# PacificBiosciences/portello

Measured on AMD Instinct MI355X. Metric: lifted HiFi reads/sec (whole node), higher is better.
Workload: dtype int32; 1 GPU; wgs30x; reads_total=2000000, reads_this_rank=2000000, read_len_mean=15000, items_per_gpu=2065417, in_ops_per_gpu=62827345, out_ops_per_gpu=56590310, large_items_per_gpu=0, mid_items_per_gpu=0, retry_items_per_gpu=0, lane_items_per_gpu=2065417, heavy_lane_items_per_gpu=0, seq_fmt=bam4, parallelism=one read set, 20 Mb windows dealt to 1 ranks by input ops, gather=none, launched_by=single process

## Files before the change

portello_amd/csrc/lane_core.hpp:

```cpp
#pragma once
#include <plo_wave.hpp>
#include <stdint.h>

#include <type_traits>
#ifdef PLO_EMULATOR
#include <stdio.h>
#include <stdlib.h>
#endif

#include "lift_core.hpp"

#ifdef PLO_EMULATOR
#define PLO_MARK(s)
#else
#define PLO_MARK(s) asm volatile("; " s)
#endif

namespace plo {



#ifdef PLO_EMULATOR
struct __attribute__((packed, aligned(4))) Ops4 {
    uint32_t x, y, z, w;
};
#else
typedef uint32_t Ops4 __attribute__((ext_vector_type(4), aligned(4)));
#endif
struct LaneOut {
    uint32_t *R = nullptr;
    int no = 0;
    uint32_t acc = 0;
    int lead_shift = 0;
    bool seen_m = false;
    bool pairs = false;
    bool ovf = false;
    uint16_t *H = nullptr;
    int extra = 0;
};
PLO_DEV int wrap_add(int a, int b) { return (int)((unsigned)a + (unsigned)b); }
PLO_DEV bool b_is_match(int t) { return ((0x181u >> t) & 1u) != 0u; }
PLO_DEV bool b_is_indel(int t) { return (unsigned)(t - 1) < 2u; }
PLO_DEV bool b_ref_cons(int t) { return ((0x18Du >> t) & 1u) != 0u; }
PLO_DEV bool b_read_cons(int t) { return ((0x1B3u >> t) & 1u) != 0u; }

constexpr int H16_MAX = 8191, H16_CHUNKS = 8;
constexpr int H16_ALLOW = 4;
PLO_DEV uint32_t h16_dec(uint32_t h) { return ((h >> 3) << 4) | (h & 7u); }
PLO_DEV uint32_t h16_enc(int t, uint32_t len) { return (len << 3) | (uint32_t)t; }

template <int ST, bool H16>
PLO_DEV void lane_flush(LaneOut &o, bool flush, int wlim) {
    const int at = (int)(o.acc & 15u);
    if constexpr (!H16) {
        const bool ok = o.no < wlim;
        if (flush & ok) o.R[o.no * ST] = o.acc;
        o.ovf = o.ovf | (flush & !ok);
        o.no += flush ? 1 : 0;
    } else {
        static_assert(ST == 1, "H16 regions are lane-contiguous");
        const uint32_t len = o.acc >> 4;
        const bool ok = o.no < wlim;
        if (flush & ok) o.H[o.no] = (uint16_t)h16_enc(at, len < (uint32_t)H16_MAX ? len : (uint32_t)H16_MAX);
        o.ovf = o.ovf | (flush & !ok);
        o.no += flush ? 1 : 0;
        const bool big = flush & (len > (uint32_t)H16_MAX);
        if (wv::ballot(big) != 0ull) {
            uint32_t rest = big ? len - (uint32_t)H16_MAX : 0u;
#pragma unroll
            for (int c = 1; c < H16_CHUNKS; ++c) {
                const bool more = rest > 0u;
                const uint32_t part = rest < (uint32_t)H16_MAX ? rest : (uint32_t)H16_MAX;
                const bool okc = o.no < wlim;
                if (more & okc) o.H[o.no] = (uint16_t)h16_enc(at, part);
                o.ovf = o.ovf | (more & !okc);
                o.no += more ? 1 : 0;
                o.extra += more ? 1 : 0;
                rest -= part;
            }
            o.ovf = o.ovf | (rest > 0u);
        }
    }
}
template <bool PAD = true, int ST = 1, bool H16 = false>
PLO_DEV void lane_push(LaneOut &o, bool on, int t, int L, int wlim) {
    if constexpr (ST != 1) on = on & !o.ovf;
    const bool lead = on & !o.seen_m;
    const bool drop_d = lead & (t == OP_D);
    o.lead_shift += drop_d ? L : 0;
    t = (lead & (t == OP_I)) ? (int)OP_S : t;
    o.seen_m = o.seen_m | (on & b_is_match(t));
    const bool live = on & !drop_d & (L > 0);
    const int at = (int)(o.acc & 15u);
    const bool same = live & (t == at);
    const bool flush = live & !same & (o.acc >= 16u);
    o.pairs = o.pairs | (flush & b_is_indel(at) & b_is_indel(t));
    lane_flush<ST, H16>(o, flush, wlim);
    const uint32_t add = (PAD && t == OP_P) ? 0u : ((uint32_t)L << 4);
    o.acc = same ? o.acc + add : (live ? mk_op(t, L) : o.acc);
}
template <bool H16 = false>
PLO_DEV void lane_out_finish(LaneOut &o, bool on, int wlim) {
    lane_flush<1, H16>(o, on & (o.acc >= 16u), wlim);
    const bool fix0 = on & !o.ovf & o.seen_m;
    if constexpr (H16) {
        int lm = o.no - 1;
        {
            bool look = fix0 & (lm >= 0);
            while (wv::ballot(look) != 0ull) {
                const uint32_t c = o.H[look ? lm : 0];
                const bool hit = look & b_is_match((int)(c & 7u));
                look = look & !hit & (lm > 0);
                lm -= (look) ? 1 : 0;
            }
        }
        const bool fix = fix0 & (lm + 1 < o.no);
        LaneOut o2;
        o2.H = o.H;
        o2.no = lm + 1;
        o2.seen_m = true;
        int i = lm + 1, cont = 0, prev_t = -1;
        while (wv::ballot(fix & (i < o.no)) != 0ull) {
            const bool act = fix & (i < o.no);
            const uint32_t c = h16_dec(o.H[act ? i : 0]);
            int t = op_type(c);
            const int L = op_len(c);
            i += act ? 1 : 0;
            cont += (act & (t == prev_t)) ? 1 : 0;
            prev_t = act ? t : prev_t;
            const bool keep = act & (t != OP_D);
            t = (t == OP_I) ? (int)OP_S : t;
            lane_push<true, 1, true>(o2, keep, t, L, i);
        }
        lane_flush<1, true>(o2, fix & (o2.acc >= 16u), o.no);
        o.no = fix ? o2.no : o.no;
        o.extra = fix ? o.extra - cont + o2.extra : o.extra;
    } else {
        int lm = o.no - 1;
        {
            bool look = fix0 & (lm >= 0);
            while (wv::ballot(look) != 0ull) {
                const uint32_t c = o.R[look ? lm : 0];
                const bool hit = look & b_is_match(op_type(c));
                look = look & !hit & (lm > 0);
                lm -= (look) ? 1 : 0;
            }
        }
        const bool fix = fix0 & (lm + 1 < o.no);
        int i = lm + 1, w = lm + 1;
        uint32_t run = 0;
        while (wv::ballot(fix & (i < o.no)) != 0ull) {
            const bool act = fix & (i < o.no);
            const uint32_t c = o.R[act ? i : 0];
            int t = op_type(c);
            const int L = op_len(c);
            i += act ? 1 : 0;
            const bool keep = act & (t != OP_D);
            t = (t == OP_I) ? (int)OP_S : t;
            const bool same = keep & (run >= 16u) & (t == (int)(run & 15u));
            const bool flush = keep & !same & (run >= 16u);
            if (flush) o.R[w] = run;
            w += flush ? 1 : 0;
            const uint32_t add = (t == OP_P) ? 0u : ((uint32_t)L << 4);
            run = same ? run + add : (keep ? mk_op(t, L) : run);
        }
        {
            const bool flush = fix & (run >= 16u);
            if (flush) o.R[w] = run;
            w += flush ? 1 : 0;
            o.no = fix ? w : o.no;
        }
    }
}

struct XW16 {
    Ops4 r4, q4;
    uint32_t r1, q1;
    int rsh, qsh, jmin;
};
PLO_DEV bool xw16_issue(bool on, const uint8_t *ref, int ref_len, int r0, const ReadSeq &rd, int q0, const uint8_t *safe, XW16 &w, bool &miss) {
    bool ok = on & (r0 >= 0) & (q0 >= 0) & (q0 <= rd.len - 16);
    const int rsh = (int)(((unsigned)(uintptr_t)ref + (unsigned)r0) & 3u);
    ok = ok & (r0 - rsh >= 0) & (r0 - rsh <= ref_len - 20);
    const int jmin = rd.flip ? rd.len - q0 - 16 : q0;
    const bool bam4 = rd.fmt != PLO_SEQ_ASCII;
    int b0 = bam4 ? (jmin >> 1) : jmin;
    miss = false;
    if (rd.fmt == PLO_SEQ_BAM4_SPARSE) {
        const int j0 = ok ? jmin : 0, j1 = ok ? jmin + 15 : 0;
        const int g0 = j0 >> 5, g1 = j1 >> 5;
        const PLO_GLOBAL uint32_t *hdr = (const PLO_GLOBAL uint32_t *)(ok ? rd.p : safe);
        const uint32_t m0 = hdr[2 * (g0 >> 5)], rk0 = hdr[2 * (g0 >> 5) + 1], m1 = hdr[2 * (g1 >> 5)];
        const bool present = (((m0 >> (g0 & 31)) & (m1 >> (g1 & 31))) & 1u) != 0u;
        const unsigned rank = rk0 + (unsigned)__builtin_popcount(m0 & ((1u << (g0 & 31)) - 1u));
        const long long off = (long long)rd.data + (long long)rank * 16 + ((j0 >> 1) & 15);
        const bool bad = !present | (rank > 0x3ffffffu) | (off + (g1 - g0) * 16 + 20 > (long long)rd.hi);
        miss = ok & bad;
        ok = ok & !bad;
        b0 = (int)off;
    }
    const int qsh = (int)(((unsigned)(uintptr_t)rd.p + (unsigned)b0) & 3u);
    ok = ok & (b0 - qsh >= rd.lo) & (b0 - qsh + 20 <= rd.hi);
#ifdef PLO_EXP_PROBE_NOMEM
    const PLO_GLOBAL uint32_t *pr = (const PLO_GLOBAL uint32_t *)safe;
    const PLO_GLOBAL uint32_t *pq = (const PLO_GLOBAL uint32_t *)safe;
#else
    const PLO_GLOBAL uint32_t *pr = (const PLO_GLOBAL uint32_t *)(ok ? ref + (r0 - rsh) : safe);
    const PLO_GLOBAL uint32_t *pq = (const PLO_GLOBAL uint32_t *)(ok ? rd.p + (b0 - qsh) : safe);
#endif
    w.r4 = *(const PLO_GLOBAL Ops4 *)pr;
    w.r1 = pr[4];
    w.q4 = *(const PLO_GLOBAL Ops4 *)pq;
    w.q1 = pq[4];
    w.rsh = rsh;
    w.qsh = qsh;
    w.jmin = jmin;
    return ok;
}
PLO_DEV void xw16_decode(const ReadSeq &rd, const XW16 &wx, unsigned X[4]) {
    struct {
        unsigned wr[5], wq[5];
        int rsh, qsh, jmin;
    } w = {{wx.r4.x, wx.r4.y, wx.r4.z, wx.r4.w, wx.r1}, {wx.q4.x, wx.q4.y, wx.q4.z, wx.q4.w, wx.q1}, wx.rsh, wx.qsh, wx.jmin};
    const bool bam4 = rd.fmt != PLO_SEQ_ASCII;
    unsigned D[4];
    if (bam4) {
        unsigned S[5];
#pragma unroll
        for (int q = 0; q < 3; ++q) {
            unsigned Q = wv::align_bytes(w.wq[q + 1], w.wq[q], (unsigned)w.qsh);
            unsigned H = (Q >> 4) & 0x0f0f0f0fu, L = Q & 0x0f0f0f0fu;
            S[2 * q] = wv::perm_bytes(L, H, 0x05010400u);
            if (2 * q + 1 < 5) S[2 * q + 1] = wv::perm_bytes(L, H, 0x07030602u);
        }
        const unsigned par = (unsigned)(w.jmin & 1);
        const unsigned long long lo = rd.flip ? 0x4e4e4e434e47544eull : 0x565352474d43413dull;
        const unsigned long long hi = rd.flip ? 0x4e4e4e4e4e4e4e41ull : 0x4e42444b48595754ull;
#pragma unroll
        for (int v = 0; v < 4; ++v) {
            unsigned T = wv::align_bytes(S[v + 1], S[v], par);
            unsigned idx = T & 0x07070707u;
            unsigned dl = wv::perm_bytes((unsigned)(lo >> 32), (unsigned)lo, idx);
            unsigned dh = wv::perm_bytes((unsigned)(hi >> 32), (unsigned)hi, idx);
            unsigned mk = ((T >> 3) & 0x01010101u) * 0xffu;
            D[v] = (dh & mk) | (dl & ~mk);
        }
    } else {
#pragma unroll
        for (int v = 0; v < 4; ++v) {
            D[v] = wv::align_bytes(w.wq[v + 1], w.wq[v], (unsigned)w.qsh);
            if (rd.flip) D[v] = comp4(D[v]);
        }
    }
#pragma unroll
    for (int u = 0; u < 4; ++u) {
        unsigned R = wv::align_bytes(w.wr[u + 1], w.wr[u], (unsigned)w.rsh);
        unsigned B = rd.flip ? wv::perm_bytes(0u, D[3 - u], 0x00010203u) : D[u];
        X[u] = R ^ B;
    }
}

struct LaneProbe {
    XW16 w;
    int re = 0, qe = 0, maxk = 0;
    bool async_ok = false;
    bool miss = false;
};
PLO_DEV void lane_probe_arm(LaneProbe &p, bool on, int ref_len, int rs, int del, const ReadSeq &rd, int qs, int ins, int bound, bool &panic) {
    const int re = rs + del, qe = qs + ins;
    const int max_left = wv::imin(rs, qs);
    int maxk = wv::imin(max_left, bound);
    const bool bad = (max_left > 0) & ((re - 1 >= ref_len) | (qe - 1 >= rd.len));
    panic = panic | (on & bad);
    maxk = (bad | !on) ? 0 : maxk;
    p.re = re;
    p.qe = qe;
    p.maxk = maxk;
}
PLO_DEV void lane_probe_load(LaneProbe &p, bool on, const uint8_t *ref, int ref_len, const ReadSeq &rd, const uint8_t *safe) {
    p.async_ok = xw16_issue(on & (p.maxk > 0), ref, ref_len, p.re - 16, rd, p.qe - 16, safe, p.w, p.miss);
}
PLO_DEV int match_run_back_from(const uint8_t *ref, int ref_len, int re, ReadSeq &rd, int qe, int maxk, int k, int &probes) {
    while (k < maxk) {
        unsigned X[4];
        if (!xor_window16(ref, ref_len, re - k - 16, rd, qe - k - 16, X)) break;
        int n = wv::imin(16, maxk - k);
        int m = wv::imin(zero_bytes_from_top(X), n);
        probes += wv::imin(m + 1, n);
        k += m;
        if (m < n) return k;
    }
    while (k < maxk) {
        int n = wv::imin(8, maxk - k);
        int a[8], b[8];
#pragma unroll
        for (int j = 0; j < 8; ++j) {
            int jj = j < n ? j : 0;
            a[j] = ((const PLO_GLOBAL uint8_t *)ref)[re - 1 - k - jj];
            b[j] = read_base(rd, qe - 1 - k - jj);
        }
        int adv = n;
#pragma unroll
        for (int j = 7; j >= 0; --j)
            if (j < n && a[j] != b[j]) adv = j;
        probes += wv::imin(adv + 1, n);
        k += adv;
        if (adv < n) break;
    }
    return k;
}
PLO_DEV int top_zero_bytes(const unsigned X[4]) {
    const unsigned long long hi = ((unsigned long long)X[3] << 32) | X[2], lo = ((unsigned long long)X[1] << 32) | X[0];
    const int zh = hi ? (__builtin_clzll(hi) >> 3) : 8, zl = lo ? (__builtin_clzll(lo) >> 3) : 8;
    return hi ? zh : 8 + zl;
}
PLO_DEV int lane_probe_finish(const LaneProbe &p, bool on, const uint8_t *ref, int ref_len, ReadSeq &rd, int &probes) {
    unsigned X[4];
    xw16_decode(rd, p.w, X);
    const int n = wv::imin(16, p.maxk);
    const int m = wv::imin(top_zero_bytes(X), n);
    rd.miss = rd.miss | (on & p.miss);
    const bool live = on & (p.maxk > 0) & !p.miss;
    const bool fast = live & p.async_ok;
    int h = fast ? m : 0;
    probes += fast ? wv::imin(m + 1, n) : 0;
    const bool more = live & ((!p.async_ok) | ((m == n) & (n < p.maxk)));
    if (wv::ballot(more) != 0ull) {
        if (more) h = match_run_back_from(ref, ref_len, p.re, rd, p.qe, p.maxk, h, probes);
    }
    return h;
}

constexpr int LANE_RW = 20, LANE_WW = 28;
constexpr int LANE_WIN_DWORDS = LANE_RW + LANE_WW;
constexpr int LANE_WIN_MARGIN = 8;
constexpr int LANE_REGION_PAD = LANE_RW + 4;
struct LaneWin {
    uint32_t *G = nullptr;
    uint32_t *rw = nullptr, *ww = nullptr;
    int rbase = 0, wbase = 0;
};
PLO_DEV void win_fill(LaneWin &w, bool on, int idx) {
    if (on) {
        w.rbase = idx;
        Ops4 v[LANE_RW / 4];
#pragma unroll
        for (int q = 0; q < LANE_RW / 4; ++q) v[q] = *(const PLO_GLOBAL Ops4 *)(w.G + idx + 4 * q);
#pragma unroll
        for (int q = 0; q < LANE_RW / 4; ++q) {
            w.rw[(4 * q) * 64] = v[q].x;
            w.rw[(4 * q + 1) * 64] = v[q].y;
            w.rw[(4 * q + 2) * 64] = v[q].z;
            w.rw[(4 * q + 3) * 64] = v[q].w;
        }
    }
}
PLO_DEV void win_fill_input(LaneWin &w, bool on, int idx, const uint32_t *src, int n_in, bool rev, int lo_ok, int hi_ok) {
    uint32_t a[LANE_RW];
    const uint32_t *qa[LANE_RW / 4];
    bool edge = false;
#pragma unroll
    for (int q = 0; q < LANE_RW / 4; ++q) {
        const int kq = idx + 4 * q;
        const bool want = on & (kq < n_in);
        const int gi = rev ? n_in - 4 - kq : kq;
        const bool inside = (gi >= lo_ok) & (gi + 4 <= hi_ok);
        edge = edge | (want & !inside);
        qa[q] = (want & inside) ? src + gi : (const uint32_t *)plo_safe_words;
    }
    if (wv::ballot(edge) == 0ull) {
        Ops4 v[LANE_RW / 4];
#pragma unroll
        for (int q = 0; q < LANE_RW / 4; ++q) v[q] = *(const PLO_GLOBAL Ops4 *)qa[q];
#pragma unroll
        for (int q = 0; q < LANE_RW / 4; ++q) {
            a[4 * q] = rev ? v[q].w : v[q].x;
            a[4 * q + 1] = rev ? v[q].z : v[q].y;
            a[4 * q + 2] = rev ? v[q].y : v[q].z;
            a[4 * q + 3] = rev ? v[q].x : v[q].w;
        }
    } else {
#pragma unroll
        for (int j = 0; j < LANE_RW; ++j) {
            a[j] = 0u;
            if (on && idx + j < n_in) a[j] = src[rev ? n_in - 1 - idx - j : idx + j];
        }
    }
    if (on) {
        w.rbase = idx;
#pragma unroll
        for (int j = 0; j < LANE_RW; ++j) w.rw[j * 64] = (idx + j < n_in) ? a[j] : 0u;
    }
}
PLO_DEV void win_flush(LaneWin &w, bool on, int end) {
    if (on) {
        const int cnt = end - w.wbase;
        uint32_t *const dst = w.G + w.wbase;
#pragma unroll
        for (int q = 0; q < LANE_WW / 4; ++q) {
            Ops4 v;
            v.x = w.ww[(4 * q) * 64];
            v.y = w.ww[(4 * q + 1) * 64];
            v.z = w.ww[(4 * q + 2) * 64];
            v.w = w.ww[(4 * q + 3) * 64];
            if (4 * q + 3 < cnt) *(PLO_GLOBAL Ops4 *)(dst + 4 * q) = v;
        }
        const int n4 = cnt & ~3;
#pragma unroll
        for (int j = 0; j < 3; ++j)
            if (n4 + j < cnt) dst[n4 + j] = w.ww[(n4 + j) * 64];
        w.wbase = end;
    }
}

constexpr int LANE_KVS = 128;
constexpr int LANE_KVS_DWORDS = 2 * LANE_KVS;
constexpr int LANE_KVS_MAX = 512;
template <bool SP, bool WIN = false, bool NOSHIFT = false, bool STATS = true, bool H16 = false>
PLO_DEV void lane_tile(const DevIndex &ix, const DevBatch &bt, const DevWork &wk, uint32_t stages, uint32_t item_begin, int nit,
                       uint32_t *lds, int capw, int fixed_stride, WaveCtx &ctx, const uint32_t *list, bool have_g, uint32_t g_pre,
                       uint32_t *greg = nullptr, uint32_t *kvs = nullptr, int kvs_n = LANE_KVS) {
    static_assert(!(H16 && WIN), "16-bit ops: LDS regions only");
    const int lane = wv::lane();
    const bool has = lane < nit;
    const uint32_t g = have_g ? g_pre : (has ? list[item_begin + (uint32_t)lane] : 0u);
#ifdef PLO_PHASE_TIMING
    long long tlast = wv::clock();
#define PLO_LT(k)                     \
    {                                 \
        long long now_ = wv::clock(); \
        ctx.tph[k] += now_ - tlast;   \
        tlast = now_;                 \
    }
#define PLO_LC(k, v) ctx.tph[k] += (v);
#else
#define PLO_LT(k)
#define PLO_LC(k, v)
#endif

    int n_in = 0, n_m = 0, in_off = 0, pos1 = 0, kv0 = 0, kv1 = 0, W0 = 0, W1 = 0, seq_len = 0, shift_ref_len = 0;
    bool len_bad = false, rev = false, do_shift = false, flip = false;
    unsigned long long seq_off = 0, shift_ref = 0;
    if (has) {
        in_off = (int)wk.d.in_off[g];
        n_in = (int)wk.d.n_in[g];
        n_m = (int)wk.d.n_m[g];
        W0 = (int)wk.d.w0[g];
        W1 = (int)wk.d.w1[g];
        kv0 = (int)wk.d.kv0[g];
        kv1 = (int)wk.d.kv1[g];
        const uint32_t fl = wk.d.flags[g];
        pos1 = wk.d.pos1[g];
        seq_len = (int)wk.d.seq_len[g];
        const uint32_t read_len_in = wk.d.read_len[g];
        len_bad = read_len_in == 0xffffffffu || (uint32_t)seq_len != read_len_in;
        seq_off = wk.d.seq_off[g];
        shift_ref = wk.d.shift_ref[g];
        shift_ref_len = wk.d.shift_ref_len[g];
        rev = (fl & ITF_REV) != 0;
        flip = (fl & ITF_FLIP) != 0;
        const bool contig_fwd = (fl & ITF_CONTIG_FWD) != 0;
        do_shift = (stages & PLO_STAGE_LSHIFT) && (!(stages & PLO_STAGE_STRAND) || !contig_fwd);
    }
    const bool need_shift = do_shift;
    if constexpr (NOSHIFT) do_shift = false;
    const bool merges = do_shift || (stages & PLO_STAGE_LIFTOVER);
    const int n_ld = merges ? n_m : n_in;
    const int gap = has ? lane_region_gap(W0, W1) : 0;
    const int W = n_ld + gap + LANE_SLACK + (H16 ? H16_ALLOW : 0);
    const int W_dw = H16 ? (W + 1) >> 1 : W;

    int kvs_base = 0, kvs_cnt = 0;
    bool kv_lds = false, kvs_store = false;
    constexpr int KVS_Q = H16 ? LANE_KVS_MAX / 64 : LANE_KVS / 64;
    if constexpr (!H16) kvs_n = kvs_n < LANE_KVS ? kvs_n : LANE_KVS;
    KV kvs_e[KVS_Q];
#pragma unroll
    for (int q = 0; q < KVS_Q; ++q) kvs_e[q] = {0, 0};
    if (kvs != nullptr && (stages & PLO_STAGE_LIFTOVER)) {
        const int need_hi = wv::imin(kv1, W1 + 2);
        kvs_base = -wv::reduce_max(has ? -W0 : -IMAX);
        const int top = wv::reduce_max(has ? need_hi : 0);
        const int cnt = wv::imax(0, wv::imin(top - kvs_base, kvs_n));
        kv_lds = has & (need_hi <= kvs_base + cnt);
        kvs_cnt = cnt;
#pragma unroll
        for (int q = 0; q < KVS_Q; ++q)
            if (64 * q < kvs_n && lane + 64 * q < cnt) kvs_e[q] = ix.kv[kvs_base + lane + 64 * q];
        kvs_store = true;
    }

    bool pending = has;
    {
        const bool defer = has && (W_dw > (WIN ? fixed_stride - LANE_REGION_PAD : capw) || (NOSHIFT && need_shift));
        const unsigned long long dm = wv::ballot(defer);
        if (dm != 0ull) {
            int slot = 0;
            if (lane == 0) slot = (int)wv::atomic_add_global(&wk.counters[CNT_NRETRY], (unsigned long long)__builtin_popcountll(dm));
            slot = wv::bcast_first(slot);
            if (defer) {
                wk.retry_list[slot + __builtin_popcountll(dm & ((1ull << lane) - 1ull))] = g;
                wk.status[g] = (uint8_t)ITEM_NEED_BIG;
                pending = false;
            }
        }
    }

    while (wv::ballot(pending) != 0ull) {
        const int wv_ = pending ? W_dw : 0;
        const int incl = WIN ? 0 : wv::scan_add(wv_);
        const bool act0 = pending && (WIN || incl <= capw);
        pending = pending && !act0;
        uint32_t *R = WIN ? nullptr : lds + (act0 ? incl - wv_ : 0);
        uint16_t *const R16 = (uint16_t *)R;
        LaneWin win;
        if constexpr (WIN) {
            win.G = greg + (size_t)(has ? lane : 0) * (size_t)fixed_stride;
            win.rw = lds + lane;
            win.ww = lds + LANE_RW * 64 + lane;
        }
        wv::sync();

        int status = PLO_ITEM_LIFTED;
        bool alive = act0;
        bool shift_on = act0 && do_shift;
        if (shift_on && shift_ref == 0ull) {
            status = PLO_ITEM_PANIC;
            alive = false;
            shift_on = false;
        }
        bool ovf = false, panic = false;
        unsigned algo = 0;
        int cur_off = 0, n = 0;
        int nops = 0;
        constexpr int ST = WIN ? 64 : 1;
        auto rd_at = [&](int k, bool ok) -> uint32_t {
            if constexpr (WIN) return win.rw[ok ? (cur_off + k - win.rbase) * 64 : 0];
            else if constexpr (H16) return h16_dec(R16[cur_off + (ok ? k : 0)]);
            else return R[cur_off + (ok ? k : 0)];
        };
        const bool direct = WIN && (stages & PLO_STAGE_LIFTOVER) != 0u;
        const int n_cig_all = WIN ? (int)bt.seg_cigar_off[bt.n_segs] : 0;
        bool ext = false;
        auto rd_fill = [&](bool on, int idx) {
            if constexpr (WIN) {
                if (direct) {
                    if (wv::ballot(on & ext) != 0ull) win_fill_input(win, on & ext, idx, bt.cigar + in_off, n_in, rev, -in_off, n_cig_all - in_off);
                    if (wv::ballot(on & !ext) != 0ull) win_fill(win, on & !ext, idx);
                } else {
                    win_fill(win, on, idx);
                }
            }
        };
        auto rd_need = [&](int k, bool ok, bool stage_on) {
            if constexpr (WIN) {
                if (wv::ballot(ok & (cur_off + k - win.rbase >= LANE_RW)) != 0ull) rd_fill(stage_on, cur_off + k);
            }
        };
        auto wr_open = [&](LaneOut &o, int base) {
            if constexpr (WIN) {
                win.wbase = base;
                o.R = win.ww;
            } else if constexpr (H16) {
                o.H = R16 + base;
            } else {
                o.R = R + base;
            }
        };
        auto wr_room = [&](LaneOut &o, bool on, int base) {
            if constexpr (WIN) {
                if (wv::ballot(on & !o.ovf & (base + o.no - win.wbase > LANE_WW - LANE_WIN_MARGIN)) != 0ull) {
                    win_flush(win, on & !o.ovf, base + o.no);
                    o.R = win.ww - o.no * 64;
                }
            }
        };
        auto wr_finish = [&](LaneOut &o, bool on, int base, int wlim) {
            if constexpr (WIN) {
                win_flush(win, on & !o.ovf, base + o.no);
                o.R = win.G + base;
            }
            lane_out_finish<H16>(o, on, wlim);
        };
        int pos = pos1;
        ReadSeq rd = item_read_seq<SP>(bt, seq_off, seq_len, flip ? 1 : 0);
        PLO_LT(0)

        if (direct) {
            n = act0 ? n_in : 0;
            ext = act0;
        } else {
            const bool ld = act0;
            const bool merge = ld & merges;
            const int inb = shift_on ? W - n_ld - (H16 ? H16_ALLOW : 0) : gap;
            const int nmax = wv::reduce_max(ld ? n_in : 0);
            const int n_cig = (int)bt.seg_cigar_off[bt.n_segs];
            uint32_t run = 0;
            bool has_run = false;
            int w = 0;
            if constexpr (WIN) win.wbase = inb;
            bool ld_ovf = false;
            auto put = [&](bool on, uint32_t v) {
                if constexpr (WIN) {
                    if (on) win.ww[(inb + w - win.wbase) * 64] = v;
                } else if constexpr (H16) {
                    const uint32_t len = v >> 4;
                    const int vt = b_is_match((int)(v & 15u)) ? (int)OP_M : (int)(v & 15u);
                    const bool ok = inb + w < W;
                    if (on & ok) R16[inb + w] = (uint16_t)h16_enc(vt, len < (uint32_t)H16_MAX ? len : (uint32_t)H16_MAX);
                    ld_ovf = ld_ovf | (on & !ok);
                } else {
                    if (on) R[inb + w] = v;
                }
            };
            auto put_more = [&](bool on, uint32_t v) {
                if constexpr (H16) {
                    const uint32_t len = v >> 4;
                    const bool big = on & (len > (uint32_t)H16_MAX);
                    if (wv::ballot(big) != 0ull) {
                        uint32_t rest = big ? len - (uint32_t)H16_MAX : 0u;
#pragma unroll
                        for (int c = 1; c < H16_CHUNKS; ++c) {
                            const bool more = rest > 0u;
                            const uint32_t part = rest < (uint32_t)H16_MAX ? rest : (uint32_t)H16_MAX;
                            const bool ok = inb + w < W;
                            if (more & ok) R16[inb + w] = (uint16_t)h16_enc(b_is_match((int)(v & 15u)) ? (int)OP_M : (int)(v & 15u), part);
                            ld_ovf = ld_ovf | (more & !ok);
                            w += more ? 1 : 0;
                            rest -= part;
                        }
                        ld_ovf = ld_ovf | (rest > 0u);
                    }
                }
            };
            constexpr int LB = 16;
            for (int k0 = 0; k0 < nmax; k0 += LB) {
                PLO_LC(10, 1)
                if constexpr (WIN) {
                    if (wv::ballot(ld & (inb + w - win.wbase > LANE_WW - (LB + 1))) != 0ull) win_flush(win, ld, inb + w);
                }
                uint32_t r[LB];
                const uint32_t *qa[LB / 4];
                bool edge = false;
#pragma unroll
                for (int q = 0; q < LB / 4; ++q) {
                    const int kq = k0 + 4 * q;
                    const bool want = ld & (kq < n_in);
                    const int gi = in_off + (rev ? n_in - 4 - kq : kq);
                    const bool inside = (gi >= 0) & (gi <= n_cig - 4);
                    edge = edge | (want & !inside);
                    qa[q] = (want & inside) ? bt.cigar + gi : (const uint32_t *)plo_safe_words;
                }
                if (wv::ballot(edge) == 0ull) {
                    Ops4 v[LB / 4];
#pragma unroll
                    for (int q = 0; q < LB / 4; ++q) v[q] = *(const PLO_GLOBAL Ops4 *)qa[q];
#pragma unroll
                    for (int q = 0; q < LB / 4; ++q) {
                        r[4 * q] = rev ? v[q].w : v[q].x;
                        r[4 * q + 1] = rev ? v[q].z : v[q].y;
                        r[4 * q + 2] = rev ? v[q].y : v[q].z;
                        r[4 * q + 3] = rev ? v[q].x : v[q].w;
                    }
                } else {
#pragma unroll
                    for (int j = 0; j < LB; ++j) {
                        r[j] = 0u;
                        if (ld && k0 + j < n_in) r[j] = bt.cigar[in_off + (rev ? (n_in - 1 - k0 - j) : k0 + j)];
                    }
                }
#pragma unroll
                for (int j = 0; j < LB; ++j) {
                    const bool have = ld & (k0 + j < n_in);
                    const uint32_t c = r[j];
                    const bool join = merge & have & has_run & b_is_match(op_type(c)) & b_is_match(op_type(run));
                    const bool flush = have & has_run & !join;
                    put(flush, run);
                    w += flush ? 1 : 0;
                    put_more(flush, run);
                    run = join ? ((run & ~15u) + (c & ~15u)) | (uint32_t)OP_M : (have ? c : run);
                    has_run = has_run | have;
                }
            }
            put(ld & has_run, run);
            w += (ld & has_run) ? 1 : 0;
            put_more(ld & has_run, run);
            if constexpr (WIN) win_flush(win, ld, inb + w);
            n = ld ? w : 0;
            cur_off = ld ? inb : 0;
            if constexpr (H16) ovf = ovf | (ld & ld_ovf);
        }
        if (kvs_store) {
#pragma unroll
            for (int q = 0; q < KVS_Q; ++q)
                if (64 * q < kvs_n) {
                    kvs[2 * (lane + 64 * q)] = (uint32_t)kvs_e[q].key;
                    kvs[2 * (lane + 64 * q) + 1] = (uint32_t)kvs_e[q].val;
                }
            kvs_store = false;
        }
        wv::sync();

        PLO_LT(1)
        if constexpr (!NOSHIFT) if (wv::ballot(shift_on) != 0ull) {
            const uint8_t *const sref = (const uint8_t *)(uintptr_t)shift_ref;
            LaneOut o;
            wr_open(o, gap);
            rd_fill(shift_on, cur_off);
            const int wl0 = cur_off - gap;
            const int wl_ext = W - gap;
            int k = 0;
            bool fin = !shift_on;
            int ref_head = pos1, read_head = 0, match = 0, del = 0, ins = 0, blk_ref = 0, blk_read = 0;
            bool in_blk = false, pend = false;
            int p_match = 0, p_ins = 0, p_del = 0, msince = 0, probes = 0;
            LaneProbe pr;
            PLO_MARK("SHIFT LOOP BEGIN");
            for (unsigned long long bm; (bm = wv::ballot(!fin)) != 0ull;) {
                PLO_LC(8, 1)
                if constexpr (STATS) {
                    ctx.u_act += (unsigned)__builtin_popcountll(bm);
                    ctx.u_trips += 1;
                }
                wr_room(o, shift_on, gap);
                if (wv::ballot(pend) != 0ull) lane_probe_load(pr, pend, sref, shift_ref_len, rd, (const uint8_t *)plo_safe_words);
                bool stop = fin, ev_other = false, ev_end = false;
                int ev_t = 0, ev_L = 0;
                while (wv::ballot(!stop) != 0ull) {
                    PLO_LC(9, 1)
                    const bool act = !stop;
                    const bool have = k < n;
                    rd_need(k, have & shift_on, shift_on);
                    const uint32_t c = rd_at(k, have & (!WIN | shift_on));
                    const int t = op_type(c), L = op_len(c);
                    const bool indel = have & b_is_indel(t);
                    const bool ism = have & b_is_match(t);
                    const bool other = have & !indel & !ism;
                    const bool atend = !have;
                    const bool ev = act & ((in_blk & (ism | other | atend)) | other | atend);
                    const bool take = act & !ev;
                    const bool memb = take & indel & (L > 0);
                    const bool open = memb & !in_blk;
                    blk_ref = open ? ref_head : blk_ref;
                    blk_read = open ? read_head : blk_read;
                    in_blk = in_blk | memb;
                    del += (memb & (t == OP_D)) ? L : 0;
                    ins += (memb & (t == OP_I)) ? L : 0;
                    const bool tm = take & ism;
                    msince += (tm & pend) ? L : 0;
                    match += (tm & !pend) ? L : 0;
                    read_head += (take & b_read_cons(t)) ? L : 0;
                    ref_head += (take & b_ref_cons(t)) ? L : 0;
                    k += take ? 1 : 0;
                    ev_t = ev ? t : ev_t;
                    ev_L = ev ? L : ev_L;
                    ev_other = ev ? other : ev_other;
                    ev_end = ev ? atend : ev_end;
                    stop = stop | ev;
                }
                const bool evl = !fin;
                const bool endc = evl & in_blk;
                const bool flushing = evl & (ev_other | ev_end);
                const int wl = ext ? wl_ext : wl0 + k;
                auto resolve = [&](bool on) {
                    int h = lane_probe_finish(pr, on, sref, shift_ref_len, rd, probes);
                    h = rd.miss ? 0 : h;
                    const int sh = wv::imin(p_match, h);
                    lane_push<false, ST, H16>(o, on & (p_match - sh > 0), OP_M, p_match - sh, wl);
                    lane_push<false, ST, H16>(o, on & (p_ins > 0), OP_I, p_ins, wl);
                    lane_push<false, ST, H16>(o, on & (p_del > 0), OP_D, p_del, wl);
                    match = on ? sh + msince : match;
                    msince = on ? 0 : msince;
                    pend = pend & !on;
                };
#pragma nounroll
                for (int pass = 0; pass < 2; ++pass) {
                    const bool res = (pass == 0 ? evl : flushing) & pend;
                    if (wv::ballot(res) != 0ull) {
                        if (pass == 1) lane_probe_load(pr, res, sref, shift_ref_len, rd, (const uint8_t *)plo_safe_words);
                        resolve(res);
                    }
                    if (pass == 1) break;
                    if (wv::ballot(endc) != 0ull) {
                        lane_probe_arm(pr, endc, shift_ref_len, blk_ref, del, rd, blk_read, ins, match, panic);
                        p_match = endc ? match : p_match;
                        p_ins = endc ? ins : p_ins;
                        p_del = endc ? del : p_del;
                        ins = endc ? 0 : ins;
                        del = endc ? 0 : del;
                        in_blk = in_blk & !endc;
                        pend = pend | endc;
                    }
                    if (wv::ballot(flushing & pend) == 0ull) break;
                }
                if (wv::ballot(flushing) != 0ull) {
                    lane_push<false, ST, H16>(o, flushing & (match > 0), OP_M, match, wl);
                    match = flushing ? 0 : match;
                    const bool oth = flushing & ev_other;
                    lane_push<true, ST, H16>(o, oth, ev_t, ev_L, wl + 1);
                    read_head += (oth & b_read_cons(ev_t)) ? ev_L : 0;
                    ref_head += (oth & b_ref_cons(ev_t)) ? ev_L : 0;
                    k += oth ? 1 : 0;
                    fin = fin | (flushing & ev_end);
                }
            }
            PLO_MARK("SHIFT LOOP END");
            wr_finish(o, shift_on, gap, ext ? wl_ext : wl0 + n);
            if (shift_on) {
                if constexpr (STATS) algo += 2u * (unsigned)probes;
                n = o.no;
                cur_off = gap;
                ext = false;
                pos += o.lead_shift;
                ovf = ovf | o.ovf;
            }
        }
        if (act0 && (panic || rd.miss)) {
            status = rd.miss ? PLO_ITEM_NEED_BASES : PLO_ITEM_PANIC;
            alive = false;
        }
        wv::sync();
        PLO_LT(2)

        bool pairs = true;
        if (stages & PLO_STAGE_LIFTOVER) {
            const bool lo_on = alive && !ovf;
            if constexpr (STATS) {
                if (lo_on) {
                    const int nb = kv1 - kv0;
                    const int lg = nb > 1 ? 32 - __builtin_clz((unsigned)(nb - 1)) : 0;
                    algo += 16u * (unsigned)(W1 - W0) + 8u * (unsigned)lg;
                }
            }
            LaneOut o;
            wr_open(o, 0);
            rd_fill(lo_on, cur_off);
            int k = 0;
            bool in_op = false, ism = false, bvalid = false, has_start = false, has_end = false;
            int t = 0, seg_start = pos, seg_end = 0, block_pos = 0, r2s = 0, r2e = 0;
            int kb = 0, vb = NONE32, kn = IMAX, vn = NONE32, kf = IMAX, vf = NONE32;
            int ni = W0 + 2;
            auto run = [&](auto all_lds_c) {
                constexpr bool ALL_LDS = decltype(all_lds_c)::value;
                auto kv_fetch = [&](bool on, int idx, int &key, int &val) {
                    if (kvs != nullptr) {
                        const bool l = ALL_LDS ? on : (on & kv_lds & ((unsigned)(idx - kvs_base) < (unsigned)kvs_cnt));
#ifdef PLO_EMULATOR
                        if (ALL_LDS && on && (unsigned)(idx - kvs_base) >= (unsigned)kvs_cnt) {
                            fprintf(stderr, "lane_tile: block-map entry %d outside the staged range [%d, %d)\n", idx, kvs_base, kvs_base + kvs_cnt);
                            abort();
                        }
#endif
                        const uint32_t *q = kvs + 2 * (l ? idx - kvs_base : 0);
                        const int lk = (int)q[0], lv = (int)q[1];
                        key = l ? lk : key;
                        val = l ? lv : val;
                        on = on & !l;
                    }
                    if constexpr (!ALL_LDS) {
                        const bool gl = on;
                        if (wv::ballot(gl) != 0ull) {
                            if (gl) {
                                const KV e = ix.kv[idx];
                                key = e.key;
                                val = e.val;
                            }
                        }
                    }
                };
                kv_fetch(lo_on & (W0 < kv1), W0, kn, vn);
                kv_fetch(lo_on & (W0 + 1 < kv1), W0 + 1, kf, vf);
                PLO_MARK("LIFTOVER LOOP BEGIN");
                for (unsigned long long bm; (bm = wv::ballot(lo_on & ((k < n) | in_op))) != 0ull;) {
                    PLO_LC(7, 1)
                    if constexpr (STATS) {
                        ctx.u_act += (unsigned)__builtin_popcountll(bm);
                        ctx.u_trips += 1;
                    }
                    const bool fetch = lo_on & !in_op & (k < n);
                    wr_room(o, lo_on, 0);
                    rd_need(k, fetch, lo_on);
                    const uint32_t c = rd_at(k, fetch);
                    k += fetch ? 1 : 0;
                    const int tf = op_type(c), Lf = op_len(c);
                    const bool copy = fetch & (((0x32u >> tf) & 1u) != 0u);
                    const bool start = fetch & b_ref_cons(tf) & (Lf > 0);
                    t = start ? ((unsigned)(tf - (int)OP_D) < 2u ? tf : (int)OP_M) : t;
                    ism = start ? b_is_match(tf) : ism;
                    seg_end = start ? seg_start + Lf : seg_end;
                    block_pos = start ? seg_start : block_pos;
                    in_op = in_op | start;
                    const bool adv = in_op & (kn <= block_pos);
                    int fk = IMAX, fv = NONE32;
                    kv_fetch(adv & (ni < kv1), ni, fk, fv);
                    kb = adv ? kn : kb;
                    vb = adv ? vn : vb;
                    bvalid = bvalid | adv;
                    kn = adv ? kf : kn;
                    vn = adv ? vf : vn;
                    ni += adv ? 1 : 0;
                    const bool piece = in_op & (kn > block_pos);
                    const int pend = wv::imin(seg_end, kn);
                    const int plen = pend - block_pos;
                    const bool mapped = bvalid & (vb != NONE32);
                    const bool mp = piece & mapped;
                    const bool set_start = mp & ism & !has_start;
                    r2s = set_start ? wrap_add(vb, block_pos - kb) : r2s;
                    has_start = has_start | set_start;
                    const int d = wrap_add(vb, -r2e);
                    const bool e0 = mp & has_end & (d > 0) & has_start;
                    has_end = has_end | mp;
                    const bool go = piece & !e0;
                    r2e = mp ? wrap_add(vb, e0 ? 0 : pend - kb) : r2e;
                    const bool e1p = go & (mapped ? (ism | has_start) : ism);
                    const int t1p = mapped ? t : (bvalid ? (int)OP_I : (int)OP_S);
                    block_pos = go ? pend : block_pos;
                    const bool done = go & (pend >= seg_end);
                    in_op = in_op & !done;
                    seg_start = done ? seg_end : seg_start;
                    const int wl = ext ? W : cur_off + k;
                    lane_push<false, ST, H16>(o, e0 | copy | e1p, e0 ? (int)OP_D : (copy ? tf : t1p), e0 ? d : (copy ? Lf : plen), wl);
                    kf = adv ? fk : kf;
                    vf = adv ? fv : vf;
                }
            };
            if (kvs != nullptr && wv::ballot(lo_on & !kv_lds) == 0ull) run(std::true_type{});
            else run(std::false_type{});
            PLO_MARK("LIFTOVER LOOP END");
            PLO_LT(3)
            wr_finish(o, lo_on, 0, ext ? W : cur_off + n);
            if (lo_on) {
                ovf = ovf | o.ovf;
                if (!has_start) {
                    status = PLO_ITEM_NO_LIFTOVER;
                    alive = false;
                } else {
                    n = o.no;
                    nops = o.no - o.extra;
                    cur_off = 0;
                    ext = false;
                    pos = r2s + o.lead_shift;
                }
                pairs = o.pairs;
            }
            wv::sync();
        }

        PLO_LT(4)
        bool simp = alive && !ovf;
        if ((stages & PLO_STAGE_LENCHECK) && simp && len_bad) {
            status = PLO_ITEM_LEN_MISMATCH;
            simp = false;
        }

        if (stages & PLO_STAGE_SIMPLIFY) {
            const bool s_on = simp && (!(stages & PLO_STAGE_LIFTOVER) || pairs);
            if (wv::ballot(s_on) != 0ull) {
                unsigned long long chrom_ref = 0;
                int chrom_ref_len = 0;
                if (s_on) {
                    chrom_ref = wk.d.chrom_ref[g];
                    chrom_ref_len = wk.d.chrom_ref_len[g];
                }
                const uint8_t *const cref = (const uint8_t *)(uintptr_t)chrom_ref;
                LaneOut o;
                wr_open(o, 0);
                rd_fill(s_on, cur_off);
                int ref_head = pos, read_head = 0, del = 0, ins = 0, blk_ref = 0, blk_read = 0, cmp = 0;
                bool in_blk = false, spanic = false, zero_m = false;
                const int nmax = wv::reduce_max(s_on ? n : 0);
                for (int k = 0; k <= nmax; ++k) {
                    const bool valid = s_on & (k < n);
                    const bool atend = s_on & (k == n);
                    wr_room(o, s_on, 0);
                    rd_need(k, valid, s_on);
                    const uint32_t c = rd_at(k, valid);
                    const int t = op_type(c), L = op_len(c);
                    const bool indel = valid & b_is_indel(t);
                    const int wl = cur_off + wv::imin(k + 1, n);
                    const bool endc = in_blk & !indel & (valid | atend);
                    if (wv::ballot(endc) != 0ull) {
                        const bool single = endc & ((del == 0) | (ins == 0));
                        const bool one_one = endc & (del == 1) & (ins == 1);
                        const bool cplx = endc & !single & !one_one;
                        int pre = one_one ? 1 : 0, post = 0;
                        if (wv::ballot(cplx) != 0ull) {
                            if (cplx) {
                                if (blk_ref < 0 || blk_ref + del - 1 >= chrom_ref_len || blk_read + ins - 1 >= rd.len) {
                                    spanic = true;
                                    del = 0;
                                    ins = 0;
                                } else {
                                    post = match_run_back(cref, chrom_ref_len, blk_ref + del, rd, blk_read + ins, wv::imin(del, ins), cmp);
                                    del -= post;
                                    ins -= post;
                                    pre = match_run_fwd(cref, chrom_ref_len, blk_ref, rd, blk_read, wv::imin(del, ins), cmp);
                                    del -= pre;
                                    ins -= pre;
                                    if (del == 1 && ins == 1) {
                                        del = 0;
                                        ins = 0;
                                        ++post;
                                    }
                                }
                            }
                        }
                        const bool emit_id = endc & !one_one;
                        const bool both = wv::ballot(endc & !single) != 0ull;
                        if (both) lane_push<false, ST, H16>(o, endc & (pre > 0), OP_M, pre, wl);
                        {
                            const bool first_d = emit_id & (ins == 0);
                            lane_push<false, ST, H16>(o, emit_id & ((first_d ? del : ins) > 0), first_d ? (int)OP_D : (int)OP_I, first_d ? del : ins, wl);
                            if (both) {
                                lane_push<false, ST, H16>(o, emit_id & !first_d & (del > 0), OP_D, del, wl);
                                lane_push<false, ST, H16>(o, endc & (post > 0), OP_M, post, wl);
                            }
                        }
                        del = endc ? 0 : del;
                        ins = endc ? 0 : ins;
                        in_blk = in_blk & !endc;
                    }
                    const bool open = indel & !in_blk;
                    blk_ref = open ? ref_head : blk_ref;
                    blk_read = open ? read_head : blk_read;
                    in_blk = in_blk | indel;
                    del += (indel & (t == OP_D)) ? L : 0;
                    ins += (indel & (t == OP_I)) ? L : 0;
                    const bool cp = valid & !indel;
                    zero_m = zero_m | (cp & b_is_match(t) & (L == 0));
                    lane_push<true, ST, H16>(o, cp, t, L, wl);
                    read_head += (valid & b_read_cons(t)) ? L : 0;
                    ref_head += (valid & b_ref_cons(t)) ? L : 0;
                }
                wr_finish(o, s_on, 0, cur_off + n);
                if (s_on) {
                    if constexpr (STATS) algo += 2u * (unsigned)cmp;
                    ovf = ovf | o.ovf | zero_m;
                    n = o.no;
                    nops = o.no - o.extra;
                    cur_off = 0;
                    pos += o.lead_shift;
                    if (rd.miss || spanic) {
                        status = rd.miss ? PLO_ITEM_NEED_BASES : PLO_ITEM_PANIC;
                        alive = false;
                    }
                }
                wv::sync();
            }
        }

        PLO_LT(5)
        {
            const bool re = act0 && ovf;
            const unsigned long long om = wv::ballot(re);
            if (om != 0ull) {
                int slot = 0;
                if (lane == 0) slot = (int)wv::atomic_add_global(&wk.counters[CNT_NRETRY], (unsigned long long)__builtin_popcountll(om));
                slot = wv::bcast_first(slot);
                if (re) {
                    wk.retry_list[slot + __builtin_popcountll(om & ((1ull << lane) - 1ull))] = g;
                    wk.status[g] = (uint8_t)ITEM_NEED_BIG;
                }
            }
        }
        const bool done = act0 && !ovf;
        const bool emit_cigar = done && (status == PLO_ITEM_LIFTED || status == PLO_ITEM_LEN_MISMATCH);
        const int oc = emit_cigar ? (H16 ? nops : n) : 0;
        const int inco = wv::scan_add(oc);
        const int oS = inco - oc;
        const int total = wv::bcast_last(inco);
        if ((unsigned long long)total > ctx.slab_left) {
            const unsigned long long want = (unsigned long long)total > SLAB_OPS ? (unsigned long long)total : SLAB_OPS;
            unsigned long long nb = 0;
            if (lane == 0) nb = wv::atomic_add_global(&wk.counters[CNT_CIGAR], want) + wk.slab_offset;
            ctx.slab_base = wv::bcast_first(nb);
            ctx.slab_left = want;
        }
        const unsigned long long gbase = ctx.slab_base;
        ctx.slab_base += (unsigned long long)total;
        ctx.slab_left -= (unsigned long long)total;
        const bool fits = gbase + (unsigned long long)total <= wk.out_cap;
        if (!fits && lane == 0) wv::atomic_add_global(&wk.counters[CNT_OVERFLOW], 1ull);
        if constexpr (H16) {
            const int nh = (emit_cigar && fits) ? n : 0;
            const int nhmax = wv::reduce_max(nh);
            uint32_t *const dst = wk.out_cigar + gbase + (unsigned long long)oS;
            const uint16_t *const srcp = R16 + cur_off;
            if (wv::ballot(nh != (fits ? oc : 0)) == 0ull) {
                for (int k = 0; k < nhmax; k += 4) {
                    if (k + 3 < nh) {
                        Ops4 v;
                        v.x = h16_dec(srcp[k]);
                        v.y = h16_dec(srcp[k + 1]);
                        v.z = h16_dec(srcp[k + 2]);
                        v.w = h16_dec(srcp[k + 3]);
                        *(PLO_GLOBAL Ops4 *)(dst + k) = v;
                    } else {
#pragma unroll
                        for (int j = 0; j < 4; ++j)
                            if (k + j < nh) dst[k + j] = h16_dec(srcp[k + j]);
                    }
                }
            } else {
                uint32_t run = 0;
                int w = 0;
                for (int k = 0; k < nhmax; ++k) {
                    const bool act = k < nh;
                    const uint32_t c = h16_dec(srcp[act ? k : 0]);
                    const bool same = act & (run >= 16u) & (((c ^ run) & 15u) == 0u);
                    const bool fl = act & !same & (run >= 16u);
                    if (fl) dst[w] = run;
                    w += fl ? 1 : 0;
                    run = same ? run + (c & ~15u) : (act ? c : run);
                }
                if ((nh > 0) & (run >= 16u)) dst[w] = run;
            }
        } else {
            const int ocmax = wv::reduce_max(fits ? oc : 0);
            uint32_t *const dst = wk.out_cigar + gbase + (unsigned long long)oS;
            const uint32_t *const srcp = (WIN ? win.G : R) + cur_off;
            for (int k = 0; k < ocmax; k += 4) {
                if (fits && k + 3 < oc) {
                    Ops4 v;
                    v.x = srcp[k];
                    v.y = srcp[k + 1];
                    v.z = srcp[k + 2];
                    v.w = srcp[k + 3];
                    *(PLO_GLOBAL Ops4 *)(dst + k) = v;
                } else {
#pragma unroll
                    for (int j = 0; j < 4; ++j)
                        if (fits && k + j < oc) dst[k + j] = srcp[k + j];
                }
            }
        }
        if (done) {
            if (status == PLO_ITEM_NEED_BASES) wk.miss_list[wv::atomic_add_global(&wk.counters[CNT_NMISS], 1ull)] = g;
            wk.status[g] = (uint8_t)status;
            wk.pos[g] = emit_cigar ? (int64_t)pos : (int64_t)-1;
            wk.cig_off[g] = emit_cigar ? gbase + (unsigned long long)oS : 0ull;
            wk.cig_len[g] = (uint32_t)oc;
            if constexpr (STATS) ctx.algo_bytes += algo + 40u + 4u * (unsigned)n_in + 24u + 4u * (unsigned)oc;
            ctx.in_ops += (unsigned)n_in;
            ctx.out_ops += (unsigned)oc;
        }
        PLO_LT(6)
        PLO_LC(11, 1)
    }
#undef PLO_LT
#undef PLO_LC
}

template <bool SP, bool NOSHIFT = false, bool STATS = true, bool H16 = false>
PLO_DEV void lane_tiles_persistent(const DevIndex &ix, const DevBatch &bt, const DevWork &wk, uint32_t stages, uint32_t first, uint32_t stride,
                                   uint32_t n0, uint32_t n1, uint32_t gs, uint32_t *lds, int capw, WaveCtx &ctx, uint32_t base = 0, int kvs_n = LANE_KVS) {
    const uint32_t lane = (uint32_t)wv::lane();
    const bool listed = wk.lane_groups != nullptr;
    const uint32_t t0 = (n0 + gs - 1u) / gs, t1 = (n1 + gs - 1u) / gs;
    uint32_t n_groups = listed ? wv::bcast_first(*wk.lane_n_groups) : t0 + t1;
    if (listed && n_groups > wk.lane_groups_cap) {
        if (first == 0u && lane == 0u) wv::atomic_add_global(&wk.counters[CNT_ERROR], 1ull);
        n_groups = wk.lane_groups_cap;
    }
    auto group = [&](uint32_t t, uint32_t &lo, uint32_t &hi) {
        if (listed) {
            lo = wk.lane_groups[2 * t];
            hi = lo + wk.lane_groups[2 * t + 1];
        } else {
            bool second;
            uint32_t idx;
            if (wk.lane_tail_rounds) {
                const uint32_t keep = wk.lane_tail_rounds * stride, tail = t0 < keep ? t0 : keep;
                const uint32_t head0 = t0 - tail, head = head0 + t1;
                if (t >= head) {
                    second = false;
                    idx = head0 + (t - head);
                } else {
                    const uint32_t r0 = (uint32_t)(((unsigned long long)t * t1) / head), r1 = (uint32_t)(((unsigned long long)(t + 1u) * t1) / head);
                    second = r1 > r0;
                    idx = second ? r0 : t - r0;
                }
            } else {
                const uint32_t m = t0 < t1 ? t0 : t1;
                second = t < 2u * m ? (t & 1u) != 0u : t1 > t0;
                idx = t < 2u * m ? t >> 1 : t - m;
            }
            if (!second) {
                lo = idx * gs;
                hi = lo + gs < n0 ? lo + gs : n0;
            } else {
                lo = n0 + idx * gs;
                hi = lo + gs < n0 + n1 ? lo + gs : n0 + n1;
            }
            lo += base;
            hi += base;
        }
    };
    auto slot = [&](uint32_t j) { return j * stride + (first + j) % stride; };
    const bool dyn = wk.lane_ticket != nullptr;
    const uint32_t n_static = dyn ? (wk.lane_static_rounds ? wk.lane_static_rounds : 1u) : 0xffffffffu;
    const uint32_t t_base = dyn ? n_static * stride : 0u;
    uint32_t t = slot(0), lo = 0, hi = 0, g = 0;
    bool have = t < n_groups;
    if (have) {
        group(t, lo, hi);
        g = lo + lane < hi ? wk.perm[lo + lane] : 0u;
    }
    for (uint32_t j = 0; have; ++j) {
        const bool next_fixed = j + 1u < n_static;
        uint32_t tn = next_fixed ? slot(j + 1u) : 0xffffffffu, lon = 0, hin = 0, gn = 0, ticket = 0;
        if (next_fixed) {
            if (tn < n_groups) {
                group(tn, lon, hin);
                gn = lon + lane < hin ? wk.perm[lon + lane] : 0u;
            }
        } else if (dyn) {
            if (lane == 0u) ticket = wv::atomic_add_global(wk.lane_ticket, 1u);
        }
#ifdef PLO_PHASE_TIMING
        const long long tg0 = wv::realtime(), lt0 = ctx.tph[7], sr0 = ctx.tph[8], sc0 = ctx.tph[9], rd0 = ctx.tph[11];
#endif
        lane_tile<SP, false, NOSHIFT, STATS, H16>(ix, bt, wk, stages, lo, (int)(hi - lo), lds, capw, 0, ctx, wk.perm, true, g, nullptr, lds + capw, kvs_n);
        wv::sync();
#ifdef PLO_PHASE_TIMING
        {
            const long long dt = wv::realtime() - tg0;
            ctx.g_n += 1;
            ctx.g_max = dt > ctx.g_max ? dt : ctx.g_max;
            ctx.g_prev = ctx.g_last;
            ctx.g_last = dt;
            ctx.g_last_begin = tg0;
            if (lane == 0u && t < 49152u) {
                unsigned long long *r = wk.wave_stats + (size_t)8192 * STAT_WORDS + (size_t)t * 4;
                r[0] = (unsigned long long)dt | ((unsigned long long)(tg0 - ctx.t_begin) << 32);
                r[1] = (unsigned long long)(ctx.tph[7] - lt0) | ((unsigned long long)(ctx.tph[8] - sr0) << 32);
                r[2] = (unsigned long long)(ctx.tph[9] - sc0) | ((unsigned long long)(ctx.tph[11] - rd0) << 32);
                r[3] = (unsigned long long)lo | ((unsigned long long)(hi - lo) << 32) | ((unsigned long long)first << 44);
            }
        }
#endif
        if (!next_fixed && dyn) {
            const uint32_t k = wv::bcast_first(ticket);
            tn = k < n_groups ? k + t_base : 0xffffffffu;
            if (tn < n_groups) {
                group(tn, lon, hin);
                gn = lon + lane < hin ? wk.perm[lon + lane] : 0u;
            }
        }
        have = tn < n_groups;
        t = tn;
        lo = lon;
        hi = hin;
        g = gn;
    }
}

template <bool SP>
PLO_DEV void lane_heavy_persistent(const DevIndex &ix, const DevBatch &bt, const DevWork &wk, uint32_t stages, uint32_t first, uint32_t step,
                                   uint32_t lo, uint32_t mid, uint32_t hi, uint32_t per, uint32_t *windows, uint32_t *regions, int stride, WaveCtx &ctx) {
    const uint32_t t0 = (mid - lo + per - 1) / per, t1 = (hi - mid + per - 1) / per;
    for (uint32_t t = first; t < t0 + t1; t += step) {
        const bool c1 = t >= t0;
        const uint32_t b = c1 ? mid + (t - t0) * per : lo + t * per, e = c1 ? hi : mid;
        const uint32_t n = e - b < per ? e - b : per;
        lane_tile<SP, true>(ix, bt, wk, stages, b, (int)n, windows, 0x7fffffff, stride, ctx, wk.perm, false, 0u, regions, windows + 64 * LANE_WIN_DWORDS);
        wv::sync();
    }
}

}
```

Measured before the change: 1.488 billion reads/s.

## Add vectorized quad-load CIGAR loader for non-window 32-bit lane path

Adds a specialized load path for the non-window, 32-bit-op lane kernel. It reads input CIGAR ops in 16-byte quads, with direction-specialized variants for all-forward, all-reverse and mixed waves, and falls back to scalar loads only near buffer edges. Adjacent-op merging becomes a bitmask trick, replacing the generic put logic. It also merges the insertion and deletion pushes into one conditional push, and guards the event push with a wave ballot so uniformly inactive waves skip it. The specialization grows code size and register pressure and duplicates the load logic, and it drops the H16_ALLOW margin for this path.

```diff
diff --git a/portello_amd/csrc/lane_core.hpp b/portello_amd/csrc/lane_core.hpp
--- a/portello_amd/csrc/lane_core.hpp
+++ b/portello_amd/csrc/lane_core.hpp
@@ -438,6 +438,7 @@
 #define PLO_LC(k, v)
 #endif
 
+    PLO_MARK("GROUP PROLOGUE BEGIN");
     int n_in = 0, n_m = 0, in_off = 0, pos1 = 0, kv0 = 0, kv1 = 0, W0 = 0, W1 = 0, seq_len = 0, shift_ref_len = 0;
     bool len_bad = false, rev = false, do_shift = false, flip = false;
     unsigned long long seq_off = 0, shift_ref = 0;
@@ -506,6 +507,7 @@
         }
     }
 
+    PLO_MARK("GROUP PROLOGUE END");
     while (wv::ballot(pending) != 0ull) {
         const int wv_ = pending ? W_dw : 0;
         const int incl = WIN ? 0 : wv::scan_add(wv_);
@@ -589,6 +591,90 @@
         if (direct) {
             n = act0 ? n_in : 0;
             ext = act0;
+        } else if constexpr (!WIN && !H16) {
+            const bool ld = act0;
+            const bool mg = merges;
+            const int inb = shift_on ? W - n_ld : gap;
+            const int nmax = wv::reduce_max(ld ? n_in : 0);
+            const int n_cig = (int)bt.seg_cigar_off[bt.n_segs];
+            const bool all_fwd = wv::ballot(ld & rev) == 0ull, all_rev = wv::ballot(ld & !rev) == 0ull;
+            uint32_t *const Rin = R + inb;
+            const uint32_t mk = mg ? 0x01810181u : 0u;
+            uint32_t run = 0, mp = 0;
+            int w = -1;
+            constexpr int LB = 16;
+            PLO_MARK("LOAD LOOP BEGIN");
+            for (int k0 = 0; k0 < nmax; k0 += LB) {
+                PLO_LC(10, 1)
+                const int cnt = ld ? n_in - k0 : 0;
+                const bool act = cnt > 0;
+                const int ql = wv::imin(3, (cnt - 1) >> 2);
+                const int gi0 = in_off + (rev ? n_in - 4 - k0 : k0);
+                const int gil = gi0 + (rev ? -4 : 4) * ql;
+                const bool inside = (wv::imin(gi0, gil) >= 0) & (wv::imax(gi0, gil) <= n_cig - 4);
+                const bool edge = act & !inside;
+                const char *const p0 = (act & inside) ? (const char *)(bt.cigar + gi0) : (const char *)plo_safe_words;
+                uint32_t r[LB];
+                auto quads = [&](auto mode) {
+                    constexpr int M = decltype(mode)::value;
+                    const uint32_t rm = rev ? ~0u : 0u;
+                    Ops4 v[LB / 4];
+#pragma unroll
+                    for (int q = 0; q < LB / 4; ++q) {
+                        const unsigned ob = q <= ql ? 16u * (unsigned)q : 0u;
+                        const char *a;
+                        if constexpr (M == 0) a = p0 + ob;
+                        else if constexpr (M == 1) a = q == 0 ? p0 : (p0 - 48) + (48u - ob);
+                        else a = p0 + (long long)(int)((ob ^ rm) - rm);
+                        v[q] = *(const PLO_GLOBAL Ops4 *)a;
+                    }
+#pragma unroll
+                    for (int q = 0; q < LB / 4; ++q) {
+                        const uint32_t tx = M == 2 ? (v[q].x ^ v[q].w) & rm : 0u, ty = M == 2 ? (v[q].y ^ v[q].z) & rm : 0u;
+                        r[4 * q] = M == 1 ? v[q].w : v[q].x ^ tx;
+                        r[4 * q + 1] = M == 1 ? v[q].z : v[q].y ^ ty;
+                        r[4 * q + 2] = M == 1 ? v[q].y : v[q].z ^ ty;
+                        r[4 * q + 3] = M == 1 ? v[q].x : v[q].w ^ tx;
+                    }
+                };
+                if (wv::ballot(edge) == 0ull) {
+                    if (all_fwd) quads(std::integral_constant<int, 0>());
+                    else if (all_rev) quads(std::integral_constant<int, 1>());
+                    else quads(std::integral_constant<int, 2>());
+                } else {
+#pragma unroll
+                    for (int j = 0; j < LB; ++j) {
+                        r[j] = 0u;
+                        if (j < cnt) r[j] = bt.cigar[in_off + (rev ? (n_in - 1 - k0 - j) : k0 + j)];
+                    }
+                }
+#pragma unroll
+                for (int q = 0; q < LB / 4; ++q) {
+                    if (wv::ballot(4 * q < cnt) == 0ull) break;
+                    if (4 * q < cnt) {
+#pragma unroll
+                        for (int j = 4 * q; j < 4 * q + 4; ++j) {
+                            const bool have = j < cnt;
+                            const uint32_t c = r[j];
+                            const uint32_t m = mk >> (c & 31u);
+                            const bool join = have & (((m & mp) & 1u) != 0u);
+                            mp = m;
+                            run = join ? (run & ~15u) + (c & ~15u) : (have ? c : run);
+                            w += (have & !join) ? 1 : 0;
+#ifdef PLO_EMULATOR
+                            if ((unsigned)(inb + w) >= (unsigned)W) {
+                                fprintf(stderr, "lane_tile: LOAD stores op %d of an item at index %d of its region of %d\n", k0 + j, inb + w, W);
+                                abort();
+                            }
+#endif
+                            Rin[w] = run;
+                        }
+                    }
+                }
+            }
+            PLO_MARK("LOAD LOOP END");
+            n = ld ? w + 1 : 0;
+            cur_off = ld ? inb : 0;
         } else {
             const bool ld = act0;
             const bool merge = ld & merges;
@@ -767,8 +853,9 @@
                     h = rd.miss ? 0 : h;
                     const int sh = wv::imin(p_match, h);
                     lane_push<false, ST, H16>(o, on & (p_match - sh > 0), OP_M, p_match - sh, wl);
-                    lane_push<false, ST, H16>(o, on & (p_ins > 0), OP_I, p_ins, wl);
-                    lane_push<false, ST, H16>(o, on & (p_del > 0), OP_D, p_del, wl);
+                    const bool pi = on & (p_ins > 0), pd = on & (p_del > 0);
+                    lane_push<false, ST, H16>(o, pi | pd, pi ? (int)OP_I : (int)OP_D, pi ? p_ins : p_del, wl);
+                    if (wv::ballot(pi & pd) != 0ull) lane_push<false, ST, H16>(o, pi & pd, OP_D, p_del, wl);
                     match = on ? sh + msince : match;
                     msince = on ? 0 : msince;
                     pend = pend & !on;
@@ -797,7 +884,7 @@
                     lane_push<false, ST, H16>(o, flushing & (match > 0), OP_M, match, wl);
                     match = flushing ? 0 : match;
                     const bool oth = flushing & ev_other;
-                    lane_push<true, ST, H16>(o, oth, ev_t, ev_L, wl + 1);
+                    if (wv::ballot(oth) != 0ull) lane_push<true, ST, H16>(o, oth, ev_t, ev_L, wl + 1);
                     read_head += (oth & b_read_cons(ev_t)) ? ev_L : 0;
                     ref_head += (oth & b_ref_cons(ev_t)) ? ev_L : 0;
                     k += oth ? 1 : 0;
@@ -1050,6 +1137,7 @@
         }
 
         PLO_LT(5)
+        PLO_MARK("OUTPUT BEGIN");
         {
             const bool re = act0 && ovf;
             const unsigned long long om = wv::ballot(re);
@@ -1144,6 +1232,7 @@
             ctx.in_ops += (unsigned)n_in;
             ctx.out_ops += (unsigned)oc;
         }
+        PLO_MARK("OUTPUT END");
         PLO_LT(6)
         PLO_LC(11, 1)
     }
```

Result: no change. 1.484 billion reads/s (-0.3%).
